# fusioninfer/fusioninfer

Hardware: AMD Instinct MI355X
Metric: goodput req/s (Qwen3-8B serving, closed-loop) (higher is better)
Workload: dtype bf16; 1 GPU; model=Qwen3-8B, global_batch=256, seq_len=1152, prompt_len=1024, gen_len=128, parallelism=dp1

## Files before the change

### fusioninfer_amd/models/model.py

```python

from __future__ import annotations

import math

import torch
import torch.nn as nn

import fusioninfer_amd.ops as ops
from fusioninfer_amd.config import ModelConfig
from fusioninfer_amd.distributed import parallel_state as ps
from fusioninfer_amd.distributed.layers import (
    MergedColumnParallelLinear,
    ReplicatedLinear,
    RowParallelLinear,
)
from fusioninfer_amd.engine.metadata import AttnMetadata


class Attention(nn.Module):
    def __init__(self, cfg: ModelConfig, layer_idx: int = 0):
        super().__init__()
        self.layer_idx = layer_idx
        tp = ps.tp_world_size()
        assert cfg.num_heads % tp == 0 and cfg.num_kv_heads % tp == 0, (
            "head counts must divide TP size"
        )
        self.num_heads = cfg.num_heads // tp
        self.num_kv_heads = cfg.num_kv_heads // tp
        self.head_dim = cfg.head_dim
        self.q_size = self.num_heads * self.head_dim
        self.kv_size = self.num_kv_heads * self.head_dim
        self.scale = 1.0 / math.sqrt(self.head_dim)
        self.k_scale = 1.0
        self.v_scale = 1.0
        self.eps = cfg.rms_norm_eps
        hidden = cfg.hidden_size
        self.qkv_proj = MergedColumnParallelLinear(
            hidden,
            [
                cfg.num_heads * cfg.head_dim,
                cfg.num_kv_heads * cfg.head_dim,
                cfg.num_kv_heads * cfg.head_dim,
            ],
            bias=cfg.attention_bias,
        )
        self.o_proj = RowParallelLinear(cfg.num_heads * cfg.head_dim, hidden)
        if cfg.qk_norm:
            self.q_norm_weight = nn.Parameter(
                torch.ones(cfg.head_dim, dtype=torch.bfloat16), requires_grad=False
            )
            self.k_norm_weight = nn.Parameter(
                torch.ones(cfg.head_dim, dtype=torch.bfloat16), requires_grad=False
            )
        else:
            self.q_norm_weight = None
            self.k_norm_weight = None

    def forward(
        self,
        x,
        meta: AttnMetadata,
        kv_cache,
        cos_sin: torch.Tensor,
    ) -> torch.Tensor:
        qkv = self.qkv_proj(x)
        if meta.lora is not None:
            meta.lora.apply(self.layer_idx, "qkv", x, qkv)
        q = qkv[:, : self.q_size]
        k = qkv[:, self.q_size : self.q_size + self.kv_size]
        v = qkv[:, self.q_size + self.kv_size :]
        ops.rope_qk_norm_(
            q, k, meta.positions, cos_sin,
            self.num_heads, self.num_kv_heads, self.head_dim,
            self.q_norm_weight, self.k_norm_weight, self.eps,
        )
        k_cache, v_cache = kv_cache
        fp8_kv = k_cache.dtype == torch.float8_e4m3fn
        ks = self.k_scale if fp8_kv else 1.0
        vs = self.v_scale if fp8_kv else 1.0
        ops.reshape_and_cache(k, v, k_cache, v_cache, meta.slot_mapping,
                              1.0 / ks, 1.0 / vs)
        scale = self.scale * ks

        T = qkv.shape[0]
        np_, nd = meta.num_prefill_tokens, meta.num_decode_tokens
        out = torch.empty(T, self.q_size, dtype=qkv.dtype, device=qkv.device)
        if np_ > 0:
            o = ops.prefill_attention_paged(
                q[:np_].view(np_, self.num_heads, self.head_dim),
                k_cache,
                v_cache,
                meta.prefill_block_tables,
                meta.cu_seqlens,
                meta.prefill_seq_lens_k,
                scale,
                tile_seq=meta.tile_seq,
                tile_row0=meta.tile_row0,
                tile_rows=meta.tile_rows or None,
            )
            out[:np_] = o.view(np_, self.q_size)
        if nd > 0:
            o = ops.paged_attention_decode(
                q[np_:].view(nd, self.num_heads, self.head_dim),
                k_cache,
                v_cache,
                meta.block_tables,
                meta.seq_lens,
                scale,
            )
            out[np_:] = o.view(nd, self.q_size)
        if vs != 1.0:
            out *= vs
        if meta.lora is not None:
            return self.o_proj.forward_with_lora(out, meta.lora,
                                                 self.layer_idx, "o")
        return self.o_proj(out)


class MLP(nn.Module):
    def __init__(self, cfg: ModelConfig, layer_idx: int = 0):
        super().__init__()
        self.layer_idx = layer_idx
        self.fp8 = cfg.quantization == "fp8"
        self.gate_up_proj = MergedColumnParallelLinear(
            cfg.hidden_size, [cfg.intermediate_size, cfg.intermediate_size]
        )
        self.down_proj = RowParallelLinear(cfg.intermediate_size, cfg.hidden_size)
        self.inter_per_rank = cfg.intermediate_size // ps.tp_world_size()

    def forward(self, x, lora=None) -> torch.Tensor:
        gu = self.gate_up_proj(x)
        if self.fp8:
            return self.down_proj(ops.silu_and_mul_fp8(gu))
        if lora is not None:
            lora.apply(self.layer_idx, "gate_up", x, gu)
        act = ops.silu_and_mul(gu)
        if lora is not None:
            return self.down_proj.forward_with_lora(
                act, lora, self.layer_idx, "down"
            )
        return self.down_proj(act)


class MoEMLP(nn.Module):

    def __init__(self, cfg: ModelConfig, layer_idx: int = 0):
        super().__init__()
        self.layer_idx = layer_idx
        tp = ps.tp_world_size()
        E = cfg.num_experts
        assert E % tp == 0, "num_experts must divide TP size (EP sharding)"
        self.num_experts = E
        self.top_k = cfg.num_experts_per_tok
        self.norm_topk = cfg.norm_topk_prob
        self.e_start = ps.tp_rank() * (E // tp)
        self.e_end = self.e_start + E // tp
        self.fp8 = cfg.quantization == "fp8"
        H, inter = cfg.hidden_size, cfg.moe_intermediate_size
        base = torch.initial_seed() % (2**62)
        dev = torch.empty(0).device
        gen = torch.Generator(device="cpu")
        gen.manual_seed(base)
        self.router_weight = nn.Parameter(
            (torch.randn(E, H, generator=gen, device="cpu") * 0.02)
            .to(dtype=torch.bfloat16, device=dev),
            requires_grad=False,
        )
        if dev.type == "cuda":
            egen = torch.Generator(device=dev)
            edev = dev
        else:
            egen = gen
            edev = "cpu"
        if self.fp8:
            from fusioninfer_amd.quantization import quantize_weight_fp8

            gu8, gus, dn8, dns = [], [], [], []
            for e in range(self.e_start, self.e_end):
                egen.manual_seed(base + 7919 * (e + 1))
                g_w = torch.randn(2 * inter, H, generator=egen,
                                  device=edev) * 0.02
                d_w = torch.randn(H, inter, generator=egen,
                                  device=edev) * 0.02
                w8, s = quantize_weight_fp8(g_w)
                gu8.append(w8)
                gus.append(s)
                w8, s = quantize_weight_fp8(d_w)
                dn8.append(w8)
                dns.append(s)
            self.gate_up_fp8 = nn.Parameter(
                torch.stack(gu8).to(dev), requires_grad=False
            )
            self.down_fp8 = nn.Parameter(
# ... 434 lines not shown
```

### fusioninfer_amd/ops/__init__.py

```python

from __future__ import annotations

import math
from typing import Optional

import torch

from fusioninfer_amd.ops import reference as ref

_C = None
_C_IMPORT_ERROR: Optional[BaseException] = None
try:
    import importlib

    _C = importlib.import_module("fusioninfer_amd.ops._C")
except Exception as e:
    _C_IMPORT_ERROR = e


def has_native() -> bool:
    return _C is not None


def _require_native():
# ... 41 lines not shown
        out = torch.empty(x.shape, dtype=torch.float8_e4m3fn, device=x.device)
        scales = torch.empty(x.shape[0], dtype=torch.float32, device=x.device)
        _C.rms_norm_fp8(out, scales, x, weight, eps)
        return out, scales
    return ref.rms_norm_fp8(x, weight, eps)


def fused_add_rms_norm_fp8(x, residual, weight, eps: float):
    if x.is_cuda:
        _require_native()
        out = torch.empty(x.shape, dtype=torch.float8_e4m3fn, device=x.device)
        scales = torch.empty(x.shape[0], dtype=torch.float32, device=x.device)
        _C.fused_add_rms_norm_fp8(out, scales, x, residual, weight, eps)
        return out, scales, residual
    return ref.fused_add_rms_norm_fp8(x, residual, weight, eps)


def silu_and_mul_fp8(x: torch.Tensor):
    if x.is_cuda:
        _require_native()
        inter = x.shape[-1] // 2
        out = torch.empty(
            (*x.shape[:-1], inter), dtype=torch.float8_e4m3fn, device=x.device
        )
        scales = torch.empty(x.shape[0], dtype=torch.float32, device=x.device)
        _C.silu_and_mul_fp8(out, scales, x)
        return out, scales
    return ref.silu_and_mul_fp8(x)


def quant_fp8_rows(x: torch.Tensor):
    if x.is_cuda:
        _require_native()
        out = torch.empty(x.shape, dtype=torch.float8_e4m3fn, device=x.device)
        scales = torch.empty(x.shape[0], dtype=torch.float32, device=x.device)
        _C.quant_fp8_rows(out, scales, x)
        return out, scales
    return ref.quant_fp8_rows(x)



def rope_qk_norm_(
    q: torch.Tensor,
    k: torch.Tensor,
    positions: torch.Tensor,
    cos_sin: torch.Tensor,
    num_q_heads: int,
    num_kv_heads: int,
    head_dim: int,
    q_weight: Optional[torch.Tensor] = None,
    k_weight: Optional[torch.Tensor] = None,
    eps: float = 1e-6,
):
    if q.is_cuda:
        _require_native()
        _C.rope_qk_norm(
            q, k, q_weight, k_weight, cos_sin, positions,
            num_q_heads, num_kv_heads, head_dim, eps,
        )
        return q, k
    qv = q.view(-1, num_q_heads, head_dim)
    kv = k.view(-1, num_kv_heads, head_dim)
    qo, ko = ref.rope_qk_norm(qv, kv, positions.long(), cos_sin, q_weight, k_weight, eps)
    q.copy_(qo.reshape(q.shape))
    k.copy_(ko.reshape(k.shape))
    return q, k



def reshape_and_cache(k, v, k_cache, v_cache, slot_mapping,
                      k_inv_scale: float = 1.0, v_inv_scale: float = 1.0):
    if k.is_cuda:
        _require_native()
        _C.reshape_and_cache(k, v, k_cache, v_cache, slot_mapping,
                             k_inv_scale, v_inv_scale)
        return
    H, D = k_cache.shape[1], k_cache.shape[3]
    ref.reshape_and_cache(
        k.view(-1, H, D), v.view(-1, H, D), k_cache, v_cache,
        slot_mapping.long(), k_inv_scale, v_inv_scale,
    )


def gather_kv_blocks(k_cache, v_cache, block_ids) -> torch.Tensor:
    if k_cache.is_cuda:
        _require_native()
        n = int(block_ids.numel())
        staging = torch.empty(
            (2, n, *k_cache.shape[1:]), dtype=k_cache.dtype, device=k_cache.device
        )
        _C.gather_kv_blocks(staging, k_cache, v_cache, block_ids)
        return staging
    return ref.gather_kv_blocks(k_cache, v_cache, block_ids.long())


def scatter_kv_blocks(staging, k_cache, v_cache, block_ids):
    if k_cache.is_cuda:
        _require_native()
        _C.scatter_kv_blocks(staging, k_cache, v_cache, block_ids)
        return
    ref.scatter_kv_blocks(staging, k_cache, v_cache, block_ids.long())



DECODE_PARTITION_TOKENS = 512


def paged_attention_decode(
    q: torch.Tensor,
    k_cache: torch.Tensor,
    v_cache: torch.Tensor,
    block_tables: torch.Tensor,
    seq_lens: torch.Tensor,
    scale: Optional[float] = None,
) -> torch.Tensor:
    if scale is None:
        scale = 1.0 / math.sqrt(q.shape[-1])
    if q.is_cuda:
        _require_native()
        S, Hq, D = q.shape
        out = torch.empty(q.shape, dtype=q.dtype, device=q.device)
        max_tokens = int(block_tables.shape[1]) * int(k_cache.shape[2])
        num_parts = max(
            (max_tokens + DECODE_PARTITION_TOKENS - 1) // DECODE_PARTITION_TOKENS,
            1,
        )
        ml_ws = acc_ws = None
        if num_parts > 1:
            ml_ws = torch.empty(
                (S, Hq, num_parts, 2), dtype=torch.float32, device=q.device
            )
            acc_ws = torch.empty(
                (S, Hq, num_parts, D), dtype=torch.float32, device=q.device
            )
        _C.paged_attention_decode(
            out, q, k_cache, v_cache, block_tables, seq_lens,
            ml_ws, acc_ws, num_parts, scale,
        )
        return out
    return ref.paged_attention_decode(q, k_cache, v_cache, block_tables, seq_lens, scale)


import os as _os

PREFILL_TILE_ROWS = (4 if _os.environ.get("FI_PF_NW", "8").startswith("4")
                     else 8) * 32


def prefill_tile_rows(seq_lens) -> int:
    if seq_lens and max(seq_lens) >= 4096:
        return 128
    return PREFILL_TILE_ROWS


def build_prefill_tiles(seq_lens, device=None, rows=None):
    rows = rows or PREFILL_TILE_ROWS
    tile_seq, tile_row0 = [], []
    for s, L in enumerate(seq_lens):
        for r0 in range(0, L, rows):
            tile_seq.append(s)
            tile_row0.append(r0)
    return (
        torch.tensor(tile_seq, dtype=torch.int32, device=device),
        torch.tensor(tile_row0, dtype=torch.int32, device=device),
    )


def prefill_attention(
    q: torch.Tensor,
    k: torch.Tensor,
    v: torch.Tensor,
    cu_seqlens: torch.Tensor,
    scale: Optional[float] = None,
    tile_seq: Optional[torch.Tensor] = None,
    tile_row0: Optional[torch.Tensor] = None,
    tile_rows: Optional[int] = None,
) -> torch.Tensor:
    if scale is None:
        scale = 1.0 / math.sqrt(q.shape[-1])
    if q.is_cuda:
        _require_native()
        if tile_seq is None:
            lens = (cu_seqlens[1:] - cu_seqlens[:-1]).tolist()
            tile_rows = tile_rows or prefill_tile_rows(lens)
            tile_seq, tile_row0 = build_prefill_tiles(
                lens, device=q.device, rows=tile_rows
            )
        out = torch.empty(q.shape, dtype=q.dtype, device=q.device)
        _C.prefill_attention(out, q, k, v, tile_seq, tile_row0, cu_seqlens,
                             scale, tile_rows or PREFILL_TILE_ROWS)
        return out
    return ref.prefill_attention(q, k, v, cu_seqlens, scale, causal=True)


def prefill_attention_paged(
    q: torch.Tensor,
    k_cache: torch.Tensor,
    v_cache: torch.Tensor,
    block_tables: torch.Tensor,
    cu_seqlens_q: torch.Tensor,
    seq_lens_k: torch.Tensor,
    scale: Optional[float] = None,
    tile_seq: Optional[torch.Tensor] = None,
    tile_row0: Optional[torch.Tensor] = None,
    tile_rows: Optional[int] = None,
) -> torch.Tensor:
    if scale is None:
        scale = 1.0 / math.sqrt(q.shape[-1])
    if q.is_cuda:
        _require_native()
        if tile_seq is None:
            lens = (cu_seqlens_q[1:] - cu_seqlens_q[:-1]).tolist()
            tile_rows = tile_rows or prefill_tile_rows(lens)
            tile_seq, tile_row0 = build_prefill_tiles(
                lens, device=q.device, rows=tile_rows
            )
        out = torch.empty(q.shape, dtype=q.dtype, device=q.device)
        _C.prefill_attention_paged(
            out, q, k_cache, v_cache, tile_seq, tile_row0, cu_seqlens_q,
            block_tables, seq_lens_k, scale,
            tile_rows or PREFILL_TILE_ROWS,
        )
        return out
    return ref.prefill_attention_paged(
        q, k_cache, v_cache, block_tables, cu_seqlens_q, seq_lens_k, scale
    )



def pack_moe_weights(w: torch.Tensor) -> torch.Tensor:
    E, K, N = w.shape
    assert K % 32 == 0 and N % 16 == 0, (K, N)
    return (
        w.view(E, K // 32, 4, 8, N // 16, 16)
        .permute(0, 1, 4, 2, 5, 3)
        .reshape(E, K // 32, N // 16, 64, 8)
        .contiguous()
    )


def moe_gemm(out, a, b_packed, sorted_ids, expert_ids, n_valid,
             block_m: int, gate_up: bool):
    if out.is_cuda:
        _require_native()
        _C.moe_gemm(out, a, b_packed, sorted_ids, expert_ids, n_valid,
                    block_m, gate_up)
        return out
    return ref.moe_gemm(out, a, b_packed, sorted_ids, expert_ids, n_valid,
                        block_m, gate_up)


def moe_gemm_fp8(out, a, a_scales, b_packed, b_scales, sorted_ids,
                 expert_ids, n_valid, block_m: int, gate_up: bool):
    if out.is_cuda:
        _require_native()
        _C.moe_gemm_fp8(out, a, a_scales, b_packed, b_scales, sorted_ids,
                        expert_ids, n_valid, block_m, gate_up)
        return out
    return ref.moe_gemm_fp8(out, a, a_scales, b_packed, b_scales,
                            sorted_ids, expert_ids, n_valid, block_m,
                            gate_up)


def moe_align(topi: torch.Tensor, e_start: int, e_end: int, block_m: int):
    _require_native()
    T, k = topi.shape
    n = T * k
    E_local = e_end - e_start
    PM = ((n + block_m - 1) // block_m + E_local) * block_m
    dev = topi.device
    sorted_ids = torch.empty(PM, dtype=torch.int32, device=dev)
    expert_ids = torch.empty(PM // block_m, dtype=torch.int32, device=dev)
    n_valid = torch.empty(1, dtype=torch.int32, device=dev)
    pos = torch.empty(n, dtype=torch.int32, device=dev)
    _C.moe_align(topi.reshape(-1).int().contiguous(), sorted_ids,
                 expert_ids, n_valid, pos, k, e_start, e_end, block_m)
    return sorted_ids, expert_ids, n_valid, pos, PM


def moe_router_topk(logits: torch.Tensor, k: int, renorm: bool):
    _require_native()
    T, E = logits.shape
    topv = torch.empty(T, k, dtype=torch.float32, device=logits.device)
    topi = torch.empty(T, k, dtype=torch.int32, device=logits.device)
    _C.moe_router_topk(logits.contiguous(), topv, topi, k, renorm)
    return topv, topi


def moe_combine(out, y, pos, w):
    if out.is_cuda:
        _require_native()
        _C.moe_combine(out, y, pos, w)
        return out
    return ref.moe_combine(out, y, pos, w)



LORA_MAX_RANK = 128


def lora_shapes_supported(K: int, N: int, R: int) -> bool:
    return (K % 64 == 0 and N % 16 == 0 and R % 16 == 0
            and 16 <= R <= LORA_MAX_RANK)


def lora_apply(out, x, slot_ids, a_stack, b_stack, scales):
    T, K = x.shape
    N = out.shape[1]
    S, R = a_stack.shape[0], a_stack.shape[1]
# ... 64 lines not shown
```

### fusioninfer_amd/ops/csrc/ops.hip

```cpp

#include <torch/extension.h>

#include <c10/hip/HIPStream.h>
#include <hip/hip_runtime.h>

#include "common.h"

namespace fi {

template <bool FUSED_ADD, bool FP8_OUT>
void launch_rms_norm(void*, float*, const u16*, u16*, const u16*, float, int,
                     int, hipStream_t);
void launch_silu_and_mul(u16*, const u16*, int64_t, int, hipStream_t);
template <bool SILU_MUL>
void launch_row_quant_fp8(unsigned char*, float*, const u16*, int, int,
                          hipStream_t);
void launch_rope_qk_norm(u16*, u16*, int64_t, int64_t, const u16*, const u16*,
                         const float*, const int*, int, int, int, int, float,
                         hipStream_t);
void launch_reshape_and_cache(const u16*, const u16*, void*, void*,
                              const int*, int64_t, int64_t, int, int, int,
                              int, bool, float, float, hipStream_t);
template <bool GATHER>
void launch_kv_block_copy(u16*, u16*, u16*, const int*, int, int64_t,
                          hipStream_t);
void launch_paged_attn_decode(u16*, float*, float*, const u16*, const void*,
                              const void*, const int*, const int*, int,
                              int64_t, int, int, int, int, int, float, bool,
                              hipStream_t);
void launch_prefill_attn(u16*, const u16*, const void*, const void*,
                         const int*, const int*, const int*, const int*,
                         const int*, int, int, int64_t, int64_t, int64_t, int,
                         int, int, float, bool, int, hipStream_t);
void launch_moe_gemm(u16*, const u16*, const u16*, const int*, const int*,
                     const int*, int, int, int, int, bool, hipStream_t);
void launch_moe_gemm_fp8(u16*, const unsigned char*, const float*,
                         const unsigned char*, const float*, const int*,
                         const int*, const int*, int, int, int, int, bool,
                         hipStream_t);
void launch_moe_align(const int*, int*, int*, int*, int*, int, int, int,
                      int, int, int, hipStream_t);
void launch_moe_router_topk(const float*, float*, int*, int, int, int,
                            bool, hipStream_t);
void launch_moe_combine(u16*, const u16*, const int*, const float*, int, int,
                        int, hipStream_t);
void launch_lora_apply(u16*, u16*, const u16*, const int*, const u16*,
                       const u16*, const float*, int, int, int, int, int,
                       hipStream_t);
void launch_sample_tokens(int64_t*, const float*, const float*, const int*,
                          const float*, const float*, const int64_t*, int,
                          int, hipStream_t);

}

namespace {

using fi::u16;

#define CHECK_BF16_CUDA(t)                                     \
  TORCH_CHECK((t).is_cuda(), #t " must be on GPU");            \
  TORCH_CHECK((t).scalar_type() == at::kBFloat16, #t " must be bf16")

u16* bf16_ptr(at::Tensor& t) { return reinterpret_cast<u16*>(t.data_ptr()); }
const u16* bf16_cptr(const at::Tensor& t) {
  return reinterpret_cast<const u16*>(t.data_ptr());
}

hipStream_t current_stream() {
  return c10::hip::getCurrentHIPStream().stream();
}

bool cache_is_fp8(const at::Tensor& t) {
  TORCH_CHECK(
      t.scalar_type() == at::kBFloat16 || t.scalar_type() == at::kFloat8_e4m3fn,
      "kv cache must be bf16 or float8_e4m3fn");
  return t.scalar_type() == at::kFloat8_e4m3fn;
}

void rms_norm(at::Tensor out, at::Tensor input, at::Tensor weight, double eps) {
  CHECK_BF16_CUDA(out);
  CHECK_BF16_CUDA(input);
  TORCH_CHECK(input.is_contiguous() && out.is_contiguous());
  const int hidden = input.size(-1);
  const int tokens = input.numel() / hidden;
  fi::launch_rms_norm<false, false>(bf16_ptr(out), nullptr, bf16_cptr(input),
                                    nullptr, bf16_cptr(weight),
                                    static_cast<float>(eps), tokens, hidden,
                                    current_stream());
}

void fused_add_rms_norm(at::Tensor input, at::Tensor residual,
                        at::Tensor weight, double eps) {
  CHECK_BF16_CUDA(input);
  CHECK_BF16_CUDA(residual);
  TORCH_CHECK(input.is_contiguous() && residual.is_contiguous());
  const int hidden = input.size(-1);
  const int tokens = input.numel() / hidden;
  fi::launch_rms_norm<true, false>(bf16_ptr(input), nullptr, bf16_cptr(input),
                                   bf16_ptr(residual), bf16_cptr(weight),
                                   static_cast<float>(eps), tokens, hidden,
                                   current_stream());
}

#define CHECK_FP8_OUT(o, s)                                                  \
  TORCH_CHECK((o).scalar_type() == at::kFloat8_e4m3fn && (o).is_cuda() &&    \
// ... 25 lines not shown
  fi::launch_rms_norm<true, true>(
      out.data_ptr(), out_scales.data_ptr<float>(), bf16_cptr(input),
      bf16_ptr(residual), bf16_cptr(weight), static_cast<float>(eps), tokens,
      hidden, current_stream());
}

void silu_and_mul_fp8(at::Tensor out, at::Tensor out_scales, at::Tensor input) {
  CHECK_BF16_CUDA(input);
  CHECK_FP8_OUT(out, out_scales);
  TORCH_CHECK(input.is_contiguous());
  const int inter = out.size(-1);
  TORCH_CHECK(input.size(-1) == 2 * inter);
  TORCH_CHECK(inter % 8 == 0);
  fi::launch_row_quant_fp8<true>(
      static_cast<unsigned char*>(out.data_ptr()),
      out_scales.data_ptr<float>(), bf16_cptr(input),
      input.numel() / (2 * inter), inter, current_stream());
}

void quant_fp8_rows(at::Tensor out, at::Tensor out_scales, at::Tensor input) {
  CHECK_BF16_CUDA(input);
  CHECK_FP8_OUT(out, out_scales);
  TORCH_CHECK(input.is_contiguous());
  const int cols = input.size(-1);
  TORCH_CHECK(cols % 8 == 0);
  fi::launch_row_quant_fp8<false>(
      static_cast<unsigned char*>(out.data_ptr()),
      out_scales.data_ptr<float>(), bf16_cptr(input), input.numel() / cols,
      cols, current_stream());
}

void silu_and_mul(at::Tensor out, at::Tensor input) {
  CHECK_BF16_CUDA(out);
  CHECK_BF16_CUDA(input);
  TORCH_CHECK(input.is_contiguous() && out.is_contiguous());
  const int inter = out.size(-1);
  TORCH_CHECK(input.size(-1) == 2 * inter);
  TORCH_CHECK(inter % 8 == 0);
  fi::launch_silu_and_mul(bf16_ptr(out), bf16_cptr(input),
                          input.numel() / (2 * inter), inter,
                          current_stream());
}

void rope_qk_norm(at::Tensor q, at::Tensor k,
                  c10::optional<at::Tensor> q_weight,
                  c10::optional<at::Tensor> k_weight, at::Tensor cos_sin,
                  at::Tensor positions, int64_t num_q_heads,
                  int64_t num_kv_heads, int64_t head_dim, double eps) {
  CHECK_BF16_CUDA(q);
  CHECK_BF16_CUDA(k);
  TORCH_CHECK(cos_sin.scalar_type() == at::kFloat && cos_sin.is_cuda());
  TORCH_CHECK(positions.scalar_type() == at::kInt && positions.is_cuda());
  TORCH_CHECK(q.dim() == 2 && k.dim() == 2);
  TORCH_CHECK(q.stride(1) == 1 && k.stride(1) == 1);
  const int tokens = q.size(0);
  fi::launch_rope_qk_norm(
      bf16_ptr(q), bf16_ptr(k), q.stride(0), k.stride(0),
      q_weight ? bf16_cptr(*q_weight) : nullptr,
      k_weight ? bf16_cptr(*k_weight) : nullptr, cos_sin.data_ptr<float>(),
      positions.data_ptr<int>(), tokens, num_q_heads, num_kv_heads, head_dim,
      static_cast<float>(eps), current_stream());
}

void reshape_and_cache(at::Tensor k, at::Tensor v, at::Tensor k_cache,
                       at::Tensor v_cache, at::Tensor slot_mapping,
                       double k_inv_scale, double v_inv_scale) {
  CHECK_BF16_CUDA(k);
  CHECK_BF16_CUDA(v);
  const bool fp8 = cache_is_fp8(k_cache);
  TORCH_CHECK(slot_mapping.scalar_type() == at::kInt);
  TORCH_CHECK(k.dim() == 2 && v.dim() == 2);
  TORCH_CHECK(k.stride(1) == 1 && v.stride(1) == 1);
  const int kv_heads = k_cache.size(1);
  const int block_size = k_cache.size(2);
  const int head_dim = k_cache.size(3);
  fi::launch_reshape_and_cache(
      bf16_cptr(k), bf16_cptr(v), k_cache.data_ptr(), v_cache.data_ptr(),
      slot_mapping.data_ptr<int>(), k.stride(0), v.stride(0), k.size(0),
      kv_heads, block_size, head_dim, fp8,
      static_cast<float>(k_inv_scale), static_cast<float>(v_inv_scale),
      current_stream());
}

void gather_kv_blocks(at::Tensor staging, at::Tensor k_cache,
                      at::Tensor v_cache, at::Tensor block_ids) {
  TORCH_CHECK(staging.is_cuda() &&
              staging.scalar_type() == k_cache.scalar_type());
  TORCH_CHECK(block_ids.scalar_type() == at::kInt);
  const int n = block_ids.size(0);
  const int64_t block_elems = k_cache.size(1) * k_cache.size(2) *
      k_cache.size(3) * k_cache.element_size() / 2;
  fi::launch_kv_block_copy<true>(
      static_cast<fi::u16*>(staging.data_ptr()),
      static_cast<fi::u16*>(k_cache.data_ptr()),
      static_cast<fi::u16*>(v_cache.data_ptr()), block_ids.data_ptr<int>(), n,
      block_elems, current_stream());
}

void scatter_kv_blocks(at::Tensor staging, at::Tensor k_cache,
                       at::Tensor v_cache, at::Tensor block_ids) {
  TORCH_CHECK(staging.is_cuda() &&
              staging.scalar_type() == k_cache.scalar_type());
  TORCH_CHECK(block_ids.scalar_type() == at::kInt);
  const int n = block_ids.size(0);
  const int64_t block_elems = k_cache.size(1) * k_cache.size(2) *
      k_cache.size(3) * k_cache.element_size() / 2;
  fi::launch_kv_block_copy<false>(
      static_cast<fi::u16*>(staging.data_ptr()),
      static_cast<fi::u16*>(k_cache.data_ptr()),
      static_cast<fi::u16*>(v_cache.data_ptr()), block_ids.data_ptr<int>(), n,
      block_elems, current_stream());
}

void paged_attention_decode(at::Tensor out, at::Tensor q, at::Tensor k_cache,
                            at::Tensor v_cache, at::Tensor block_tables,
                            at::Tensor seq_lens,
                            c10::optional<at::Tensor> ml_ws,
                            c10::optional<at::Tensor> acc_ws,
                            int64_t num_parts, double scale) {
  CHECK_BF16_CUDA(out);
  CHECK_BF16_CUDA(q);
  const bool fp8 = cache_is_fp8(k_cache);
  TORCH_CHECK(block_tables.scalar_type() == at::kInt &&
              block_tables.is_contiguous());
  TORCH_CHECK(seq_lens.scalar_type() == at::kInt);
  TORCH_CHECK(q.dim() == 3);
  const int num_seqs = q.size(0);
  const int num_heads = q.size(1);
  const int head_dim = q.size(2);
  const int num_kv_heads = k_cache.size(1);
  TORCH_CHECK(k_cache.size(2) == 16, "cache block_size must be 16");
  TORCH_CHECK(q.stride(2) == 1 && q.stride(1) == head_dim);
  float* ml = nullptr;
  float* acc = nullptr;
  if (num_parts > 1) {
    TORCH_CHECK(ml_ws && acc_ws, "workspace required when num_parts > 1");
    ml = ml_ws->data_ptr<float>();
    acc = acc_ws->data_ptr<float>();
  }
  fi::launch_paged_attn_decode(
      bf16_ptr(out), ml, acc, bf16_cptr(q), k_cache.data_ptr(),
      v_cache.data_ptr(), block_tables.data_ptr<int>(),
      seq_lens.data_ptr<int>(), num_seqs, q.stride(0), block_tables.size(1),
      num_kv_heads, head_dim, num_heads / num_kv_heads,
      static_cast<int>(num_parts), static_cast<float>(scale), fp8,
      current_stream());
}

void prefill_attention(at::Tensor out, at::Tensor q, at::Tensor k,
                       at::Tensor v, at::Tensor tile_seq, at::Tensor tile_row0,
                       at::Tensor cu_seqlens, double scale,
                       int64_t tile_rows) {
  TORCH_CHECK(tile_rows == 128 || tile_rows == 256,
              "tile_rows must be 128 or 256");
  CHECK_BF16_CUDA(out);
  CHECK_BF16_CUDA(q);
  TORCH_CHECK(tile_seq.scalar_type() == at::kInt &&
              tile_row0.scalar_type() == at::kInt &&
              cu_seqlens.scalar_type() == at::kInt);
  TORCH_CHECK(q.dim() == 3 && k.dim() == 3 && v.dim() == 3);
  const int num_q_heads = q.size(1);
  const int head_dim = q.size(2);
  const int num_kv_heads = k.size(1);
  TORCH_CHECK(q.stride(2) == 1 && q.stride(1) == head_dim);
  TORCH_CHECK(k.stride(2) == 1 && k.stride(1) == head_dim);
  TORCH_CHECK(v.stride(2) == 1 && v.stride(1) == head_dim);
  fi::launch_prefill_attn(
      bf16_ptr(out), bf16_cptr(q), bf16_cptr(k), bf16_cptr(v),
      tile_seq.data_ptr<int>(), tile_row0.data_ptr<int>(),
      cu_seqlens.data_ptr<int>(), nullptr, nullptr, 0, tile_seq.size(0),
      q.stride(0), k.stride(0), v.stride(0), num_q_heads, num_kv_heads,
      head_dim, static_cast<float>(scale), false,
      static_cast<int>(tile_rows / 32), current_stream());
}

void prefill_attention_paged(at::Tensor out, at::Tensor q, at::Tensor k_cache,
                             at::Tensor v_cache, at::Tensor tile_seq,
                             at::Tensor tile_row0, at::Tensor cu_seqlens,
                             at::Tensor block_tables, at::Tensor seq_lens_k,
                             double scale, int64_t tile_rows) {
  TORCH_CHECK(tile_rows == 128 || tile_rows == 256,
              "tile_rows must be 128 or 256");
  CHECK_BF16_CUDA(out);
  CHECK_BF16_CUDA(q);
  const bool fp8 = cache_is_fp8(k_cache);
  TORCH_CHECK(tile_seq.scalar_type() == at::kInt &&
              tile_row0.scalar_type() == at::kInt &&
              cu_seqlens.scalar_type() == at::kInt &&
              block_tables.scalar_type() == at::kInt &&
              seq_lens_k.scalar_type() == at::kInt);
  TORCH_CHECK(block_tables.is_contiguous());
  TORCH_CHECK(q.dim() == 3);
  const int num_q_heads = q.size(1);
  const int head_dim = q.size(2);
  const int num_kv_heads = k_cache.size(1);
  TORCH_CHECK(k_cache.size(2) == 16, "cache block_size must be 16");
  TORCH_CHECK(q.stride(2) == 1 && q.stride(1) == head_dim);
  fi::launch_prefill_attn(
      bf16_ptr(out), bf16_cptr(q), k_cache.data_ptr(), v_cache.data_ptr(),
      tile_seq.data_ptr<int>(), tile_row0.data_ptr<int>(),
      cu_seqlens.data_ptr<int>(), block_tables.data_ptr<int>(),
      seq_lens_k.data_ptr<int>(), block_tables.size(1), tile_seq.size(0),
      q.stride(0), 0, 0, num_q_heads, num_kv_heads, head_dim,
      static_cast<float>(scale), fp8,
      static_cast<int>(tile_rows / 32), current_stream());
}

struct MoeGemmDims {
  int K, N, max_mtiles;
};

MoeGemmDims check_moe_gemm(const at::Tensor& out, const at::Tensor& a,
                           const at::Tensor& b_packed,
                           const at::Tensor& sorted_ids,
                           const at::Tensor& expert_ids,
                           const at::Tensor& n_valid, int64_t block_m,
                           bool gate_up) {
  TORCH_CHECK(sorted_ids.scalar_type() == at::kInt &&
              expert_ids.scalar_type() == at::kInt &&
              n_valid.scalar_type() == at::kInt);
  TORCH_CHECK(block_m == 16 || block_m == 128, "block_m must be 16 or 128");
  const int K = a.size(1);
  const int N = out.size(1);
  const int PM = out.size(0);
  TORCH_CHECK(PM % block_m == 0, "padded rows must be block_m-aligned");
  TORCH_CHECK(K % 32 == 0, "K must be a multiple of 32");
  TORCH_CHECK(
      N % (block_m == 16 ? 64 : (gate_up ? 64 : 128)) == 0,
      "N tile misalignment");
  TORCH_CHECK(b_packed.dim() == 5 && b_packed.size(1) == K / 32 &&
              b_packed.size(2) == (gate_up ? 2 * N : N) / 16 &&
              b_packed.size(3) == 64 && b_packed.size(4) == 8,
              "b_packed layout mismatch");
  TORCH_CHECK(expert_ids.size(0) >= PM / block_m);
  if (gate_up) TORCH_CHECK(sorted_ids.size(0) >= PM);
  return {K, N, static_cast<int>(PM / block_m)};
}

void moe_gemm(at::Tensor out, at::Tensor a, at::Tensor b_packed,
              at::Tensor sorted_ids, at::Tensor expert_ids,
              at::Tensor n_valid, int64_t block_m, bool gate_up) {
  CHECK_BF16_CUDA(out);
  CHECK_BF16_CUDA(a);
  CHECK_BF16_CUDA(b_packed);
  TORCH_CHECK(out.is_contiguous() && a.is_contiguous() &&
              b_packed.is_contiguous());
  const MoeGemmDims d = check_moe_gemm(out, a, b_packed, sorted_ids,
                                       expert_ids, n_valid, block_m, gate_up);
  fi::launch_moe_gemm(bf16_ptr(out), bf16_cptr(a),
                      bf16_cptr(b_packed), sorted_ids.data_ptr<int>(),
                      expert_ids.data_ptr<int>(), n_valid.data_ptr<int>(),
                      d.max_mtiles, d.K, d.N, static_cast<int>(block_m),
                      gate_up, current_stream());
}

void moe_gemm_fp8(at::Tensor out, at::Tensor a, at::Tensor a_scales,
                  at::Tensor b_packed, at::Tensor b_scales,
                  at::Tensor sorted_ids, at::Tensor expert_ids,
                  at::Tensor n_valid, int64_t block_m, bool gate_up) {
  CHECK_BF16_CUDA(out);
  TORCH_CHECK(a.scalar_type() == at::kFloat8_e4m3fn && a.is_cuda() &&
              a.is_contiguous());
  TORCH_CHECK(b_packed.scalar_type() == at::kFloat8_e4m3fn &&
              b_packed.is_contiguous());
  TORCH_CHECK(a_scales.scalar_type() == at::kFloat &&
              b_scales.scalar_type() == at::kFloat &&
              b_scales.is_contiguous());
  const MoeGemmDims d = check_moe_gemm(out, a, b_packed, sorted_ids,
                                       expert_ids, n_valid, block_m, gate_up);
  TORCH_CHECK(b_scales.numel() ==
              b_packed.size(0) * (gate_up ? 2 * d.N : d.N));
  fi::launch_moe_gemm_fp8(
      bf16_ptr(out), static_cast<const unsigned char*>(a.data_ptr()),
      a_scales.data_ptr<float>(),
      static_cast<const unsigned char*>(b_packed.data_ptr()),
      b_scales.data_ptr<float>(), sorted_ids.data_ptr<int>(),
      expert_ids.data_ptr<int>(), n_valid.data_ptr<int>(), d.max_mtiles,
      d.K, d.N, static_cast<int>(block_m), gate_up, current_stream());
}

// ... 54 lines not shown
  CHECK_BF16_CUDA(y_ws);
  CHECK_BF16_CUDA(x);
  CHECK_BF16_CUDA(a_stack);
  CHECK_BF16_CUDA(b_stack);
  TORCH_CHECK(out.is_contiguous() && y_ws.is_contiguous() &&
              x.is_contiguous() && a_stack.is_contiguous() &&
              b_stack.is_contiguous());
  TORCH_CHECK(slot_ids.is_cuda() && slot_ids.scalar_type() == at::kInt &&
              slot_ids.is_contiguous());
  TORCH_CHECK(scales.is_cuda() && scales.scalar_type() == at::kFloat &&
              scales.is_contiguous());
  TORCH_CHECK(out.dim() == 2 && x.dim() == 2 && a_stack.dim() == 3 &&
              b_stack.dim() == 3);
  const int64_t T = x.size(0);
  const int64_t K = x.size(1);
  const int64_t N = out.size(1);
  const int64_t S = a_stack.size(0);
  const int64_t R = a_stack.size(1);
  TORCH_CHECK(T >= 1 && T < (1LL << 31) - 16 && out.size(0) == T &&
              slot_ids.numel() == T);
  TORCH_CHECK(K % 64 == 0 && N % 16 == 0 && R % 16 == 0 && R >= 16 &&
                  R <= 128,
              "lora_apply: need K % 64 == 0, N % 16 == 0, R % 16 == 0, "
              "16 <= R <= 128");
  TORCH_CHECK(a_stack.size(2) == K && b_stack.size(0) == S &&
              b_stack.size(1) == N && b_stack.size(2) == R &&
              scales.numel() == S && S >= 1);
  TORCH_CHECK(y_ws.dim() == 2 && y_ws.size(0) == T && y_ws.size(1) == R);
  fi::launch_lora_apply(bf16_ptr(out), bf16_ptr(y_ws), bf16_cptr(x),
                        slot_ids.data_ptr<int>(), bf16_cptr(a_stack),
                        bf16_cptr(b_stack), scales.data_ptr<float>(),
                        static_cast<int>(T), static_cast<int>(K),
                        static_cast<int>(N), static_cast<int>(R),
                        static_cast<int>(S), current_stream());
}

void sample_tokens(at::Tensor out, at::Tensor logits, at::Tensor temperature,
                   at::Tensor top_k, at::Tensor top_p, at::Tensor min_p,
                   at::Tensor rng) {
  TORCH_CHECK(logits.is_cuda() && logits.scalar_type() == at::kFloat &&
              logits.is_contiguous() && logits.dim() == 2,
              "sample_tokens: logits must be a contiguous [T, V] fp32 GPU "
              "tensor");
  const int64_t T = logits.size(0);
  const int64_t V = logits.size(1);
  TORCH_CHECK(T >= 1 && T < (1LL << 31) && V >= 1 && V < (1LL << 30),
              "sample_tokens: need 1 <= T < 2^31 and 1 <= V < 2^30");
  auto check_row = [&](const at::Tensor& t, at::ScalarType ty, int64_t n,
                       const char* name) {
    TORCH_CHECK(t.is_cuda() && t.scalar_type() == ty && t.is_contiguous() &&
                    t.numel() == n,
                "sample_tokens: bad ", name);
  };
  check_row(out, at::kLong, T, "out");
  check_row(temperature, at::kFloat, T, "temperature");
  check_row(top_k, at::kInt, T, "top_k");
  check_row(top_p, at::kFloat, T, "top_p");
  check_row(min_p, at::kFloat, T, "min_p");
  check_row(rng, at::kLong, 2 * T, "rng");
  fi::launch_sample_tokens(
      out.data_ptr<int64_t>(), logits.data_ptr<float>(),
      temperature.data_ptr<float>(), top_k.data_ptr<int>(),
      top_p.data_ptr<float>(), min_p.data_ptr<float>(),
      rng.data_ptr<int64_t>(), static_cast<int>(T), static_cast<int>(V),
      current_stream());
}

}

PYBIND11_MODULE(TORCH_EXTENSION_NAME, m) {
  m.def("rms_norm", &rms_norm, "RMSNorm (bf16, fp32 accum)");
  m.def("fused_add_rms_norm", &fused_add_rms_norm,
        "in-place residual add + RMSNorm");
  m.def("silu_and_mul", &silu_and_mul, "fused SiLU-mul");
  m.def("rms_norm_fp8", &rms_norm_fp8, "RMSNorm with fused fp8 row quant");
  m.def("fused_add_rms_norm_fp8", &fused_add_rms_norm_fp8,
        "residual add + RMSNorm with fused fp8 row quant");
  m.def("silu_and_mul_fp8", &silu_and_mul_fp8,
        "fused SiLU-mul with fp8 row quant");
  m.def("quant_fp8_rows", &quant_fp8_rows, "per-row dynamic fp8 quant");
  m.def("rope_qk_norm", &rope_qk_norm,
        "fused per-head qk RMSNorm + NeoX RoPE (in-place)");
  m.def("reshape_and_cache", &reshape_and_cache, "scatter K/V into paged cache");
  m.def("gather_kv_blocks", &gather_kv_blocks, "pack KV blocks for PD send");
  m.def("scatter_kv_blocks", &scatter_kv_blocks, "unpack KV blocks from PD recv");
  m.def("paged_attention_decode", &paged_attention_decode,
        "paged decode attention");
  m.def("prefill_attention", &prefill_attention, "varlen causal MFMA prefill");
  m.def("prefill_attention_paged", &prefill_attention_paged,
        "varlen causal MFMA prefill over the paged cache (context attention)");
  m.def("moe_gemm", &moe_gemm,
        "grouped MFMA GEMM over block-aligned expert segments "
        "(gate_up=true fuses the SwiGLU epilogue)");
  m.def("moe_gemm_fp8", &moe_gemm_fp8,
        "grouped fp8 (e4m3) MFMA GEMM with per-row/per-channel dequant "
        "epilogue (gate_up=true fuses SwiGLU)");
  m.def("moe_combine", &moe_combine,
        "weighted top-k combine of expert outputs (deterministic)");
  m.def("moe_align", &moe_align,
        "single-kernel block alignment of expert assignments "
        "(vLLM moe_align_block_size analog)");
  m.def("moe_router_topk", &moe_router_topk,
        "fused router tail: softmax + top-k + optional renormalize");
  m.def("lora_apply", &lora_apply,
        "batched multi-LoRA shrink + expand indexed by per-token slot ids "
        "(in-place on out)");
  m.def("sample_tokens", &sample_tokens,
        "fused temperature / top-k / top-p / min-p sampling with a "
        "counter-based (Philox4x32-10) draw, one workgroup per row");
}
```

### fusioninfer_amd/ops/csrc/rope.hip

```cpp

#include "common.h"

namespace fi {

template <int D>
__global__ void rope_qk_norm_kernel(
    u16* __restrict__ q,
    u16* __restrict__ k,
    const int64_t q_stride, const int64_t k_stride,
    const u16* __restrict__ q_weight,
    const u16* __restrict__ k_weight,
    const float* __restrict__ cos_sin,
    const int* __restrict__ positions,
    const int num_q_heads, const float eps) {
  constexpr int kHalfLanes = D / 4;
  constexpr int kActive = D / 2;
  const int lane = threadIdx.x;
  if (lane >= kActive) return;

  const int token = blockIdx.x;
  const int head = blockIdx.y;
  const bool is_q = head < num_q_heads;
  u16* base = is_q ? q + token * q_stride + static_cast<int64_t>(head) * D
                   : k + token * k_stride +
                         static_cast<int64_t>(head - num_q_heads) * D;
  const u16* w = is_q ? q_weight : k_weight;

  const int e = 2 * lane;
  u32 bits = *reinterpret_cast<const u32*>(base + e);
  float a = bf16_to_f32(static_cast<u16>(bits & 0xffff));
  float b = bf16_to_f32(static_cast<u16>(bits >> 16));

  if (w != nullptr) {
    float sumsq = a * a + b * b;
#pragma unroll
    for (int off = kActive / 2; off > 0; off >>= 1)
      sumsq += __shfl_xor(sumsq, off, 64);
    const float inv_rms = rsqrtf(sumsq / D + eps);
    const u32 wbits = *reinterpret_cast<const u32*>(w + e);
    a *= inv_rms * bf16_to_f32(static_cast<u16>(wbits & 0xffff));
    b *= inv_rms * bf16_to_f32(static_cast<u16>(wbits >> 16));
  }

  const float pa = __shfl_xor(a, kHalfLanes, 64);
  const float pb = __shfl_xor(b, kHalfLanes, 64);

  const bool is_x1 = lane < kHalfLanes;
  const int pair = is_x1 ? e : e - D / 2;
  const int pos = positions[token];
  const float2 c = *reinterpret_cast<const float2*>(
      cos_sin + static_cast<int64_t>(pos) * D + pair);
  const float2 s = *reinterpret_cast<const float2*>(
      cos_sin + static_cast<int64_t>(pos) * D + D / 2 + pair);

  float oa, ob;
  if (is_x1) {
    oa = a * c.x - pa * s.x;
    ob = b * c.y - pb * s.y;
  } else {
    oa = a * c.x + pa * s.x;
    ob = b * c.y + pb * s.y;
  }
  u32 obits = static_cast<u32>(f32_to_bf16(oa)) |
              (static_cast<u32>(f32_to_bf16(ob)) << 16);
  *reinterpret_cast<u32*>(base + e) = obits;
}

void launch_rope_qk_norm(u16* q, u16* k, int64_t q_stride, int64_t k_stride,
                         const u16* q_weight, const u16* k_weight,
                         const float* cos_sin, const int* positions,
                         int tokens, int num_q_heads, int num_kv_heads,
                         int head_dim, float eps, hipStream_t stream) {
  dim3 grid(tokens, num_q_heads + num_kv_heads), block(64);
  if (head_dim == 128) {
    hipLaunchKernelGGL((rope_qk_norm_kernel<128>), grid, block, 0, stream, q,
                       k, q_stride, k_stride, q_weight, k_weight, cos_sin,
                       positions, num_q_heads, eps);
  } else if (head_dim == 64) {
    hipLaunchKernelGGL((rope_qk_norm_kernel<64>), grid, block, 0, stream, q, k,
                       q_stride, k_stride, q_weight, k_weight, cos_sin,
                       positions, num_q_heads, eps);
  } else {
    abort();
  }
}

}
```

Measured before the change: 48.06 req/s.

## Fuse qk-norm RoPE with paged KV cache write and write attention output in place

Adds a single kernel that applies per-head RMSNorm and NeoX RoPE to q and k, writes q back in place, and stores the rotated k and the raw v directly into the paged cache. This replaces the separate rope and reshape_and_cache launches, so k is no longer written back to the qkv buffer and read again. Prefill and decode attention now also write straight into slices of the output buffer, which removes the extra copies. The new kernel uses 16-byte vectorized loads and stores with 8 elements per lane and adds stricter alignment and shape checks. Non-fp8 K in the qkv buffer is left unrotated, which is fine because only the cache is consumed afterwards.

```diff
diff --git a/fusioninfer_amd/models/model.py b/fusioninfer_amd/models/model.py
--- a/fusioninfer_amd/models/model.py
+++ b/fusioninfer_amd/models/model.py
@@ -2,6 +2,7 @@
 from __future__ import annotations
 
 import math
+import os
 
 import torch
 import torch.nn as nn
@@ -15,6 +16,8 @@
     RowParallelLinear,
 )
 from fusioninfer_amd.engine.metadata import AttnMetadata
+
+_FUSED_ROPE_CACHE = os.environ.get("FI_FUSED_ROPE_CACHE", "1") != "0"
 
 
 class Attention(nn.Module):
@@ -69,22 +72,35 @@
         q = qkv[:, : self.q_size]
         k = qkv[:, self.q_size : self.q_size + self.kv_size]
         v = qkv[:, self.q_size + self.kv_size :]
-        ops.rope_qk_norm_(
-            q, k, meta.positions, cos_sin,
-            self.num_heads, self.num_kv_heads, self.head_dim,
-            self.q_norm_weight, self.k_norm_weight, self.eps,
-        )
         k_cache, v_cache = kv_cache
         fp8_kv = k_cache.dtype == torch.float8_e4m3fn
         ks = self.k_scale if fp8_kv else 1.0
         vs = self.v_scale if fp8_kv else 1.0
-        ops.reshape_and_cache(k, v, k_cache, v_cache, meta.slot_mapping,
-                              1.0 / ks, 1.0 / vs)
+        if _FUSED_ROPE_CACHE:
+            ops.rope_qk_norm_cache_(
+                q, k, v, meta.positions, cos_sin,
+                self.num_heads, self.num_kv_heads, self.head_dim,
+                k_cache, v_cache, meta.slot_mapping,
+                self.q_norm_weight, self.k_norm_weight, self.eps,
+                1.0 / ks, 1.0 / vs,
+            )
+        else:
+            ops.rope_qk_norm_(
+                q, k, meta.positions, cos_sin,
+                self.num_heads, self.num_kv_heads, self.head_dim,
+                self.q_norm_weight, self.k_norm_weight, self.eps,
+            )
+            ops.reshape_and_cache(k, v, k_cache, v_cache, meta.slot_mapping,
+                                  1.0 / ks, 1.0 / vs)
         scale = self.scale * ks
 
         T = qkv.shape[0]
         np_, nd = meta.num_prefill_tokens, meta.num_decode_tokens
         out = torch.empty(T, self.q_size, dtype=qkv.dtype, device=qkv.device)
+        out_p = out_d = None
+        if _FUSED_ROPE_CACHE:
+            out_p = out[:np_].view(np_, self.num_heads, self.head_dim)
+            out_d = out[np_:].view(nd, self.num_heads, self.head_dim)
         if np_ > 0:
             o = ops.prefill_attention_paged(
                 q[:np_].view(np_, self.num_heads, self.head_dim),
@@ -97,8 +113,10 @@
                 tile_seq=meta.tile_seq,
                 tile_row0=meta.tile_row0,
                 tile_rows=meta.tile_rows or None,
-            )
-            out[:np_] = o.view(np_, self.q_size)
+                out=out_p,
+            )
+            if out_p is None:
+                out[:np_] = o.view(np_, self.q_size)
         if nd > 0:
             o = ops.paged_attention_decode(
                 q[np_:].view(nd, self.num_heads, self.head_dim),
@@ -107,8 +125,10 @@
                 meta.block_tables,
                 meta.seq_lens,
                 scale,
-            )
-            out[np_:] = o.view(nd, self.q_size)
+                out=out_d,
+            )
+            if out_d is None:
+                out[np_:] = o.view(nd, self.q_size)
         if vs != 1.0:
             out *= vs
         if meta.lora is not None:
diff --git a/fusioninfer_amd/ops/__init__.py b/fusioninfer_amd/ops/__init__.py
--- a/fusioninfer_amd/ops/__init__.py
+++ b/fusioninfer_amd/ops/__init__.py
@@ -147,6 +147,50 @@
     )
 
 
+def rope_qk_norm_cache_(
+    q: torch.Tensor,
+    k: torch.Tensor,
+    v: torch.Tensor,
+    positions: torch.Tensor,
+    cos_sin: torch.Tensor,
+    num_q_heads: int,
+    num_kv_heads: int,
+    head_dim: int,
+    k_cache: torch.Tensor,
+    v_cache: torch.Tensor,
+    slot_mapping: torch.Tensor,
+    q_weight: Optional[torch.Tensor] = None,
+    k_weight: Optional[torch.Tensor] = None,
+    eps: float = 1e-6,
+    k_inv_scale: float = 1.0,
+    v_inv_scale: float = 1.0,
+):
+    if q.is_cuda:
+        _require_native()
+        if head_dim not in (64, 128):
+            raise ValueError(
+                f"rope_qk_norm_cache_: head_dim must be 64 or 128, got "
+                f"{head_dim}")
+        if (k_cache.dim() != 4 or k_cache.shape != v_cache.shape
+                or k_cache.shape[1] != num_kv_heads or k_cache.shape[2] != 16
+                or k_cache.shape[3] != head_dim):
+            raise ValueError(
+                "rope_qk_norm_cache_: caches must both be "
+                f"[B, {num_kv_heads}, 16, {head_dim}], got "
+                f"{tuple(k_cache.shape)} and {tuple(v_cache.shape)}")
+        _C.rope_qk_norm_cache(
+            q, k, v, q_weight, k_weight, cos_sin, positions, k_cache,
+            v_cache, slot_mapping, num_q_heads, num_kv_heads, head_dim, eps,
+            k_inv_scale, v_inv_scale,
+        )
+        return q
+    rope_qk_norm_(q, k, positions, cos_sin, num_q_heads, num_kv_heads,
+                  head_dim, q_weight, k_weight, eps)
+    reshape_and_cache(k, v, k_cache, v_cache, slot_mapping,
+                      k_inv_scale, v_inv_scale)
+    return q
+
+
 def gather_kv_blocks(k_cache, v_cache, block_ids) -> torch.Tensor:
     if k_cache.is_cuda:
         _require_native()
@@ -169,6 +213,15 @@
 
 
 DECODE_PARTITION_TOKENS = 512
+
+
+def _check_attn_out(out: torch.Tensor, q: torch.Tensor) -> None:
+    if (out.shape != q.shape or out.dtype != q.dtype
+            or out.device != q.device or not out.is_contiguous()):
+        raise ValueError(
+            f"out must be a contiguous {tuple(q.shape)} {q.dtype} tensor on "
+            f"{q.device}, got {tuple(out.shape)} {out.dtype} strides "
+            f"{out.stride()} on {out.device}")
 
 
 def paged_attention_decode(
@@ -178,13 +231,17 @@
     block_tables: torch.Tensor,
     seq_lens: torch.Tensor,
     scale: Optional[float] = None,
+    out: Optional[torch.Tensor] = None,
 ) -> torch.Tensor:
     if scale is None:
         scale = 1.0 / math.sqrt(q.shape[-1])
+    if out is not None:
+        _check_attn_out(out, q)
     if q.is_cuda:
         _require_native()
         S, Hq, D = q.shape
-        out = torch.empty(q.shape, dtype=q.dtype, device=q.device)
+        if out is None:
+            out = torch.empty(q.shape, dtype=q.dtype, device=q.device)
         max_tokens = int(block_tables.shape[1]) * int(k_cache.shape[2])
         num_parts = max(
             (max_tokens + DECODE_PARTITION_TOKENS - 1) // DECODE_PARTITION_TOKENS,
@@ -203,7 +260,8 @@
             ml_ws, acc_ws, num_parts, scale,
         )
         return out
-    return ref.paged_attention_decode(q, k_cache, v_cache, block_tables, seq_lens, scale)
+    res = ref.paged_attention_decode(q, k_cache, v_cache, block_tables, seq_lens, scale)
+    return res if out is None else out.copy_(res)
 
 
 import os as _os
@@ -269,9 +327,12 @@
     tile_seq: Optional[torch.Tensor] = None,
     tile_row0: Optional[torch.Tensor] = None,
     tile_rows: Optional[int] = None,
+    out: Optional[torch.Tensor] = None,
 ) -> torch.Tensor:
     if scale is None:
         scale = 1.0 / math.sqrt(q.shape[-1])
+    if out is not None:
+        _check_attn_out(out, q)
     if q.is_cuda:
         _require_native()
         if tile_seq is None:
@@ -280,16 +341,18 @@
             tile_seq, tile_row0 = build_prefill_tiles(
                 lens, device=q.device, rows=tile_rows
             )
-        out = torch.empty(q.shape, dtype=q.dtype, device=q.device)
+        if out is None:
+            out = torch.empty(q.shape, dtype=q.dtype, device=q.device)
         _C.prefill_attention_paged(
             out, q, k_cache, v_cache, tile_seq, tile_row0, cu_seqlens_q,
             block_tables, seq_lens_k, scale,
             tile_rows or PREFILL_TILE_ROWS,
         )
         return out
-    return ref.prefill_attention_paged(
+    res = ref.prefill_attention_paged(
         q, k_cache, v_cache, block_tables, cu_seqlens_q, seq_lens_k, scale
     )
+    return res if out is None else out.copy_(res)
 
 
 
diff --git a/fusioninfer_amd/ops/csrc/ops.hip b/fusioninfer_amd/ops/csrc/ops.hip
--- a/fusioninfer_amd/ops/csrc/ops.hip
+++ b/fusioninfer_amd/ops/csrc/ops.hip
@@ -21,6 +21,11 @@
 void launch_reshape_and_cache(const u16*, const u16*, void*, void*,
                               const int*, int64_t, int64_t, int, int, int,
                               int, bool, float, float, hipStream_t);
+void launch_rope_qk_norm_cache(u16*, const u16*, const u16*, int64_t, int64_t,
+                               int64_t, const u16*, const u16*, const float*,
+                               const int*, void*, void*, const int*, int, int,
+                               int, int, float, bool, float, float,
+                               hipStream_t);
 template <bool GATHER>
 void launch_kv_block_copy(u16*, u16*, u16*, const int*, int, int64_t,
                           hipStream_t);
@@ -212,6 +217,72 @@
       current_stream());
 }
 
+void rope_qk_norm_cache(at::Tensor q, at::Tensor k, at::Tensor v,
+                        c10::optional<at::Tensor> q_weight,
+                        c10::optional<at::Tensor> k_weight, at::Tensor cos_sin,
+                        at::Tensor positions, at::Tensor k_cache,
+                        at::Tensor v_cache, at::Tensor slot_mapping,
+                        int64_t num_q_heads, int64_t num_kv_heads,
+                        int64_t head_dim, double eps, double k_inv_scale,
+                        double v_inv_scale) {
+  CHECK_BF16_CUDA(q);
+  CHECK_BF16_CUDA(k);
+  CHECK_BF16_CUDA(v);
+  TORCH_CHECK(head_dim == 64 || head_dim == 128,
+              "rope_qk_norm_cache: head_dim must be 64 or 128");
+  TORCH_CHECK(num_q_heads >= 1 && num_kv_heads >= 1);
+  const bool fp8 = cache_is_fp8(k_cache);
+  TORCH_CHECK(v_cache.scalar_type() == k_cache.scalar_type() &&
+              k_cache.is_cuda() && v_cache.is_cuda() &&
+              k_cache.is_contiguous() && v_cache.is_contiguous() &&
+              k_cache.dim() == 4 && v_cache.sizes() == k_cache.sizes());
+  TORCH_CHECK(k_cache.size(2) == 16, "cache block_size must be 16");
+  TORCH_CHECK(k_cache.size(1) == num_kv_heads && k_cache.size(3) == head_dim,
+              "rope_qk_norm_cache: cache must be [B, Hk, 16, D]");
+  const int64_t tokens = q.size(0);
+  TORCH_CHECK(q.dim() == 2 && k.dim() == 2 && v.dim() == 2);
+  TORCH_CHECK(q.stride(1) == 1 && k.stride(1) == 1 && v.stride(1) == 1);
+  TORCH_CHECK(q.size(1) == num_q_heads * head_dim &&
+              k.size(1) == num_kv_heads * head_dim &&
+              v.size(1) == num_kv_heads * head_dim &&
+              k.size(0) == tokens && v.size(0) == tokens);
+  TORCH_CHECK(tokens < (1LL << 31));
+  TORCH_CHECK(cos_sin.scalar_type() == at::kFloat && cos_sin.is_cuda() &&
+              cos_sin.is_contiguous() && cos_sin.dim() == 2 &&
+              cos_sin.size(1) == head_dim);
+  TORCH_CHECK(positions.scalar_type() == at::kInt && positions.is_cuda() &&
+              positions.is_contiguous() && positions.numel() == tokens);
+  TORCH_CHECK(slot_mapping.scalar_type() == at::kInt &&
+              slot_mapping.is_cuda() && slot_mapping.is_contiguous() &&
+              slot_mapping.numel() == tokens);
+  auto aligned16 = [](const at::Tensor& t) {
+    return reinterpret_cast<uintptr_t>(t.data_ptr()) % 16 == 0;
+  };
+  TORCH_CHECK(aligned16(q) && aligned16(k) && aligned16(v) &&
+                  aligned16(cos_sin) && aligned16(k_cache) &&
+                  aligned16(v_cache) && q.stride(0) % 8 == 0 &&
+                  k.stride(0) % 8 == 0 && v.stride(0) % 8 == 0,
+              "rope_qk_norm_cache: q/k/v rows and caches must be 16-byte "
+              "aligned");
+  auto weight_ptr = [&](const c10::optional<at::Tensor>& w) -> const u16* {
+    if (!w) return nullptr;
+    CHECK_BF16_CUDA(*w);
+    TORCH_CHECK(w->is_contiguous() && w->numel() == head_dim && aligned16(*w));
+    return bf16_cptr(*w);
+  };
+  const u16* qw = weight_ptr(q_weight);
+  const u16* kw = weight_ptr(k_weight);
+  fi::launch_rope_qk_norm_cache(
+      bf16_ptr(q), bf16_cptr(k), bf16_cptr(v), q.stride(0), k.stride(0),
+      v.stride(0), qw, kw, cos_sin.data_ptr<float>(),
+      positions.data_ptr<int>(), k_cache.data_ptr(), v_cache.data_ptr(),
+      slot_mapping.data_ptr<int>(), static_cast<int>(tokens),
+      static_cast<int>(num_q_heads), static_cast<int>(num_kv_heads),
+      static_cast<int>(head_dim), static_cast<float>(eps), fp8,
+      static_cast<float>(k_inv_scale), static_cast<float>(v_inv_scale),
+      current_stream());
+}
+
 void gather_kv_blocks(at::Tensor staging, at::Tensor k_cache,
                       at::Tensor v_cache, at::Tensor block_ids) {
   TORCH_CHECK(staging.is_cuda() &&
@@ -261,6 +332,8 @@
   const int num_kv_heads = k_cache.size(1);
   TORCH_CHECK(k_cache.size(2) == 16, "cache block_size must be 16");
   TORCH_CHECK(q.stride(2) == 1 && q.stride(1) == head_dim);
+  TORCH_CHECK(out.is_contiguous() && out.sizes() == q.sizes(),
+              "out must be a contiguous [S, Hq, D] tensor");
   float* ml = nullptr;
   float* acc = nullptr;
   if (num_parts > 1) {
@@ -326,6 +399,8 @@
   const int num_kv_heads = k_cache.size(1);
   TORCH_CHECK(k_cache.size(2) == 16, "cache block_size must be 16");
   TORCH_CHECK(q.stride(2) == 1 && q.stride(1) == head_dim);
+  TORCH_CHECK(out.is_contiguous() && out.sizes() == q.sizes(),
+              "out must be a contiguous [T, Hq, D] tensor");
   fi::launch_prefill_attn(
       bf16_ptr(out), bf16_cptr(q), k_cache.data_ptr(), v_cache.data_ptr(),
       tile_seq.data_ptr<int>(), tile_row0.data_ptr<int>(),
@@ -546,6 +621,8 @@
   m.def("rope_qk_norm", &rope_qk_norm,
         "fused per-head qk RMSNorm + NeoX RoPE (in-place)");
   m.def("reshape_and_cache", &reshape_and_cache, "scatter K/V into paged cache");
+  m.def("rope_qk_norm_cache", &rope_qk_norm_cache,
+        "fused qk RMSNorm + NeoX RoPE (q in place) + K/V paged-cache write");
   m.def("gather_kv_blocks", &gather_kv_blocks, "pack KV blocks for PD send");
   m.def("scatter_kv_blocks", &scatter_kv_blocks, "unpack KV blocks from PD recv");
   m.def("paged_attention_decode", &paged_attention_decode,
diff --git a/fusioninfer_amd/ops/csrc/rope.hip b/fusioninfer_amd/ops/csrc/rope.hip
--- a/fusioninfer_amd/ops/csrc/rope.hip
+++ b/fusioninfer_amd/ops/csrc/rope.hip
@@ -85,4 +85,161 @@
   }
 }
 
-}
+
+typedef u32 u32x4 __attribute__((ext_vector_type(4)));
+
+template <bool FP8>
+FI_DEV void store_cache_row(void* __restrict__ cache, const int64_t dst,
+                            const u32x4 row, const float inv_scale) {
+  if (FP8) {
+    const u32 w[4] = {row[0], row[1], row[2], row[3]};
+    float f[8];
+#pragma unroll
+    for (int j = 0; j < 8; ++j) {
+      const u16 h = static_cast<u16>(j & 1 ? w[j / 2] >> 16 : w[j / 2] & 0xffff);
+      f[j] = fminf(fmaxf(bf16_to_f32(h) * inv_scale, -448.f), 448.f);
+    }
+    u32 p[2];
+    pack_fp8x8(f, p);
+    *reinterpret_cast<uint2*>(static_cast<unsigned char*>(cache) + dst) =
+        make_uint2(p[0], p[1]);
+  } else {
+    *reinterpret_cast<u32x4*>(static_cast<u16*>(cache) + dst) = row;
+  }
+}
+
+template <int D, bool FP8>
+__global__ __launch_bounds__(256) void rope_qk_norm_cache_kernel(
+    u16* __restrict__ q,
+    const u16* __restrict__ k,
+    const u16* __restrict__ v,
+    const int64_t q_stride, const int64_t k_stride, const int64_t v_stride,
+    const u16* __restrict__ q_weight,
+    const u16* __restrict__ k_weight,
+    const float* __restrict__ cos_sin,
+    const int* __restrict__ positions,
+    void* __restrict__ k_cache,
+    void* __restrict__ v_cache,
+    const int* __restrict__ slot_mapping,
+    const int num_q_heads, const int num_kv_heads, const float eps,
+    const float k_inv_scale, const float v_inv_scale) {
+#pragma clang fp contract(off)
+  constexpr int kLanes = D / 8;
+  constexpr int kHeadsPerBlock = 256 / kLanes;
+  constexpr int kCacheBlock = 16;
+
+  const int token = blockIdx.x;
+  const int head = blockIdx.y * kHeadsPerBlock + threadIdx.x / kLanes;
+  const int sub = threadIdx.x % kLanes;
+  const int e = sub * 8;
+  if (head >= num_q_heads + 2 * num_kv_heads) return;
+
+  const bool is_q = head < num_q_heads;
+  const bool is_v = head >= num_q_heads + num_kv_heads;
+  const int kv_head =
+      is_q ? 0 : (head - num_q_heads) % num_kv_heads;
+  int64_t dst = 0;
+  if (!is_q) {
+    const int slot = slot_mapping[token];
+    if (slot < 0) return;
+    dst = ((static_cast<int64_t>(slot / kCacheBlock) * num_kv_heads +
+            kv_head) * kCacheBlock + slot % kCacheBlock) * D + e;
+  }
+
+  u16* qrow = q + token * q_stride + static_cast<int64_t>(head) * D + e;
+  const int64_t kv_off = static_cast<int64_t>(kv_head) * D + e;
+  const u16* src = is_q ? qrow
+                        : (is_v ? v + token * v_stride : k + token * k_stride) +
+                              kv_off;
+  u32x4 row = *reinterpret_cast<const u32x4*>(src);
+
+  if (!is_v) {
+    const u32 iw[4] = {row[0], row[1], row[2], row[3]};
+    float x[8];
+#pragma unroll
+    for (int j = 0; j < 4; ++j) {
+      x[2 * j] = bf16_to_f32(static_cast<u16>(iw[j] & 0xffff));
+      x[2 * j + 1] = bf16_to_f32(static_cast<u16>(iw[j] >> 16));
+    }
+
+    const u16* w = is_q ? q_weight : k_weight;
+    if (w != nullptr) {
+      float p[4];
+#pragma unroll
+      for (int j = 0; j < 4; ++j)
+        p[j] = x[2 * j] * x[2 * j] + x[2 * j + 1] * x[2 * j + 1];
+#pragma unroll
+      for (int off = kLanes / 2; off > 0; off >>= 1) {
+#pragma unroll
+        for (int j = 0; j < 4; ++j) p[j] += __shfl_xor(p[j], off, 64);
+      }
+      const float sumsq = (p[0] + p[2]) + (p[1] + p[3]);
+      const float inv_rms = rsqrtf(__builtin_fmaf(sumsq, 1.0f / D, eps));
+      const bf16x8 wv = *reinterpret_cast<const bf16x8*>(w + e);
+#pragma unroll
+      for (int j = 0; j < 8; ++j) x[j] *= inv_rms * bf16_to_f32(wv.h[j]);
+    }
+
+    float px[8];
+#pragma unroll
+    for (int j = 0; j < 8; ++j) px[j] = __shfl_xor(x[j], kLanes / 2, 64);
+
+    const bool is_x1 = sub < kLanes / 2;
+    const int pair = is_x1 ? e : e - D / 2;
+    const float* cs =
+        cos_sin + static_cast<int64_t>(positions[token]) * D + pair;
+    const float4 c0 = *reinterpret_cast<const float4*>(cs);
+    const float4 c1 = *reinterpret_cast<const float4*>(cs + 4);
+    const float4 s0 = *reinterpret_cast<const float4*>(cs + D / 2);
+    const float4 s1 = *reinterpret_cast<const float4*>(cs + D / 2 + 4);
+    const float c[8] = {c0.x, c0.y, c0.z, c0.w, c1.x, c1.y, c1.z, c1.w};
+    const float s[8] = {s0.x, s0.y, s0.z, s0.w, s1.x, s1.y, s1.z, s1.w};
+
+    u32 ow[4];
+#pragma unroll
+    for (int j = 0; j < 8; j += 2) {
+      const float m0 = px[j] * s[j];
+      const float m1 = px[j + 1] * s[j + 1];
+      const float o0 = __builtin_fmaf(x[j], c[j], is_x1 ? -m0 : m0);
+      const float o1 = __builtin_fmaf(x[j + 1], c[j + 1], is_x1 ? -m1 : m1);
+      ow[j / 2] = static_cast<u32>(f32_to_bf16(o0)) |
+                  (static_cast<u32>(f32_to_bf16(o1)) << 16);
+    }
+    row = u32x4{ow[0], ow[1], ow[2], ow[3]};
+  }
+
+  if (is_q) {
+    *reinterpret_cast<u32x4*>(qrow) = row;
+  } else {
+    store_cache_row<FP8>(is_v ? v_cache : k_cache, dst, row,
+                         is_v ? v_inv_scale : k_inv_scale);
+  }
+}
+
+void launch_rope_qk_norm_cache(
+    u16* q, const u16* k, const u16* v, int64_t q_stride, int64_t k_stride,
+    int64_t v_stride, const u16* q_weight, const u16* k_weight,
+    const float* cos_sin, const int* positions, void* k_cache, void* v_cache,
+    const int* slot_mapping, int tokens, int num_q_heads, int num_kv_heads,
+    int head_dim, float eps, bool fp8, float k_inv_scale, float v_inv_scale,
+    hipStream_t stream) {
+  if (tokens == 0) return;
+  const int heads = num_q_heads + 2 * num_kv_heads;
+  const dim3 grid(tokens, ceil_div(heads, 2048 / head_dim)), block(256);
+#define FI_ROPE_CACHE(D_, FP8_)                                             \
+  hipLaunchKernelGGL((rope_qk_norm_cache_kernel<D_, FP8_>), grid, block, 0, \
+                     stream, q, k, v, q_stride, k_stride, v_stride,         \
+                     q_weight, k_weight, cos_sin, positions, k_cache,       \
+                     v_cache, slot_mapping, num_q_heads, num_kv_heads, eps, \
+                     k_inv_scale, v_inv_scale)
+  if (head_dim == 128) {
+    if (fp8) FI_ROPE_CACHE(128, true); else FI_ROPE_CACHE(128, false);
+  } else if (head_dim == 64) {
+    if (fp8) FI_ROPE_CACHE(64, true); else FI_ROPE_CACHE(64, false);
+  } else {
+    abort();
+  }
+#undef FI_ROPE_CACHE
+}
+
+}
```

Measured after the change: 48.85 req/s (median of 6 runs). 1.6% higher.
